# USCCACS/RXMD

Hardware: AMD Instinct MI355X
Metric: MD steps/sec (RDX, 979,776 atoms/GPU; one step advances every GPU's domain: weak scaling, wall-clock steps/s of the whole job) (higher is better)
Workload: dtype f64

## Files before the change

### rxmd_amd/csrc/nonbonded.hip

```cpp
#include "engine.h"

#include <cstdlib>

namespace rxmd {

static inline int nblk(long long n, int b) { return n > 0 ? static_cast<int>((n + b - 1) / b) : 1; }
static constexpr double CEchrge = 23.02;

__global__ void k_sorted_charge(int G, const int *__restrict__ rootperm, const double *__restrict__ q, double4 *__restrict__ pk) {
  const int k = blockIdx.x * blockDim.x + threadIdx.x;
  if (k < G) pk[k].w = q[rootperm[k]];
}

__device__ inline double wave_sum_n(double v) { return wave_sum64(v); }

struct NbAcc { double f0, f1, f2, v0, v1, v2, v3, v4, v5, e11, e12; };
template <bool ENERGY>
__device__ inline void nb_pair(const DevFF &ff, const int *__restrict__ ix2, double xi, double yi, double zi, double qi, const double4 &pj, int tj, NbAcc &a) {
  const double d0 = xi - pj.x, d1 = yi - pj.y, d2 = zi - pj.z;
  const double r2 = d0 * d0 + d1 * d1 + d2 * d2;
  if (r2 > ff.rctap2) return;
  const int inxn = ix2[tj];
  const int itb = static_cast<int>(r2 * ff.UDRi);
  double t = r2 - itb * ff.UDR;
  t = t * ff.UDRi;
  const DevNBTab nd = ff.tabNB[static_cast<size_t>(inxn) * (NTABLE + 2) + itb];
  const double qij = qi * pj.w;
  const double CEvdw = nd.CEvdw + t * nd.dCEvdw_;
  const double CEclmb = (nd.CEclmb + t * nd.dCEclmb_) * qij;
  if (ENERGY) {
    a.e11 += 0.5 * (nd.Evdw + t * nd.dEvdw_);
    a.e12 += 0.5 * (nd.Eclmb + t * nd.dEclmb_) * qij;
  }
  const double c = CEvdw + CEclmb;
  a.f0 -= c * d0; a.f1 -= c * d1; a.f2 -= c * d2;
  const double hc = -0.5 * c;
  a.v0 += hc * d0 * d0; a.v1 += hc * d1 * d1; a.v2 += hc * d2 * d2; a.v3 += hc * d1 * d2; a.v4 += hc * d2 * d0; a.v5 += hc * d0 * d1;
}

#ifndef NB_UNR
#define NB_UNR 8
#endif
#ifndef NB_WPB
#define NB_WPB 8
#endif
template <bool ENERGY>
__global__ void __launch_bounds__(64 * NB_WPB) k_nonbond(int N, int S10, DevFF ff, const int *__restrict__ nb10, const int *__restrict__ n10,
                                                  const double4 *__restrict__ pk, const double *__restrict__ x, const double *__restrict__ y, const double *__restrict__ z,
                                                  const double *__restrict__ q, const int *__restrict__ type,
                                                  double *__restrict__ fx, double *__restrict__ fy, double *__restrict__ fz, double *__restrict__ pe, int assign) {
  __shared__ double sm[NB_WPB][3], sv[NB_WPB][6];
  const int lane = threadIdx.x & 63, w = __builtin_amdgcn_readfirstlane(static_cast<int>(threadIdx.x >> 6));
  if (threadIdx.x < 6 * NB_WPB) sv[threadIdx.x / 6][threadIdx.x % 6] = 0.0;
  __syncthreads();
  const int i = xcd_swizzle(blockIdx.x, gridDim.x) * (blockDim.x >> 6) + w;
  double e11 = 0.0, e12 = 0.0, e13 = 0.0;
  if (i < N) {
    const double xi = x[i], yi = y[i], zi = z[i], qi = q[i];
    const int ti = type[i];
    const int n = n10[i] & N10_COUNT;
    const size_t row = static_cast<size_t>(i) * S10;
    const int *ix2 = ff.inxn2 + ti * ff.n1;
    NbAcc acc = {0.0, 0.0, 0.0, 0.0, 0.0, 0.0, 0.0, 0.0, 0.0, 0.0, 0.0};
    for (int k0 = lane; k0 < n; k0 += 64 * NB_UNR) {
      unsigned ee[NB_UNR];
#pragma unroll
      for (int u = 0; u < NB_UNR; ++u) { const int k = k0 + 64 * u; ee[u] = (k < n) ? static_cast<unsigned>(__builtin_nontemporal_load(nb10 + row + k)) : NB10_SELF; }
#pragma unroll
      for (int u = 0; u < NB_UNR; ++u) {
        const unsigned e = ee[u];
        if (e & NB10_SELF) continue;
        nb_pair<ENERGY>(ff, ix2, xi, yi, zi, qi, pk[e & NB10_IDX_MASK], static_cast<int>((e >> NB10_IDX_BITS) & 15u), acc);
      }
    }
    e11 = acc.e11; e12 = acc.e12;
    double f0 = wave_sum_n(acc.f0), f1 = wave_sum_n(acc.f1), f2 = wave_sum_n(acc.f2);
    double v0 = acc.v0, v1 = acc.v1, v2 = acc.v2, v3 = acc.v3, v4 = acc.v4, v5 = acc.v5;
    v0 = wave_sum_n(v0); v1 = wave_sum_n(v1); v2 = wave_sum_n(v2); v3 = wave_sum_n(v3); v4 = wave_sum_n(v4); v5 = wave_sum_n(v5);
    if (lane == 0) {
      if (assign) { fx[i] = f0; fy[i] = f1; fz[i] = f2; }
      else { fx[i] += f0; fy[i] += f1; fz[i] += f2; }
      if (ENERGY) { const DevAtomP ap = ff.atom[ti]; e13 = CEchrge * (ap.chi * qi + 0.5 * ap.eta * qi * qi); }
      sv[w][0] = v0 - xi * f0; sv[w][1] = v1 - yi * f1; sv[w][2] = v2 - zi * f2; sv[w][3] = v3 - yi * f2; sv[w][4] = v4 - zi * f0; sv[w][5] = v5 - xi * f1;
    }
  }
  if (ENERGY) {
    e11 = wave_sum_n(e11); e12 = wave_sum_n(e12); e13 = wave_sum_n(e13);
    if (lane == 0) { sm[w][0] = e11; sm[w][1] = e12; sm[w][2] = e13; }
  }
  __syncthreads();
  if (ENERGY && threadIdx.x < 3) {
    double s = 0.0;
    for (int k = 0; k < NB_WPB; ++k) s += sm[k][threadIdx.x];
    if (s != 0.0) atomicAdd(pe + 11 + threadIdx.x, s);
  }
  if (threadIdx.x >= 64 && threadIdx.x < 70) {
    const int c = threadIdx.x - 64;
    double s = 0.0;
    for (int k = 0; k < NB_WPB; ++k) s += sv[k][c];
    if (s != 0.0) atomicAdd(pe + 16 + c, s);
  }
}

template <bool ENERGY>
__global__ void __launch_bounds__(64 * WIN_ROWS, 8) k_nonbond_win(int N, int G, int S10, DevFF ff, const unsigned short *__restrict__ sl10, const int *__restrict__ n10,
                                                                const int *__restrict__ rows_sorted, const int *__restrict__ win_k, const int *__restrict__ win_cnt, int maxunits,
                                                                const double4 *__restrict__ pk, const unsigned char *__restrict__ stype,
                                                                const double *__restrict__ x, const double *__restrict__ y, const double *__restrict__ z,
                                                                const double *__restrict__ q, const int *__restrict__ type,
                                                                double *__restrict__ fx, double *__restrict__ fy, double *__restrict__ fz, double *__restrict__ pe, int assign) {
  extern __shared__ double4 s_p[];
  unsigned char *s_t = reinterpret_cast<unsigned char *>(s_p + static_cast<size_t>(maxunits) * WIN_UNIT);
  __shared__ double sm[WIN_ROWS][3], sv[WIN_ROWS][6];
  constexpr int NT = 64 * WIN_ROWS;
  const int lane = threadIdx.x & 63, w = __builtin_amdgcn_readfirstlane(static_cast<int>(threadIdx.x >> 6));
  const int grp = xcd_swizzle(blockIdx.x, gridDim.x);
  const int ridx = grp * WIN_ROWS + w;
  const int i = min(rows_sorted[ridx], N);
  const int nslots = WIN_UNIT * win_cnt[grp];
  const int *wk = win_k + static_cast<size_t>(grp) * WIN_MAXUNITS;
  const int capslots = WIN_UNIT * maxunits;
  for (int t = threadIdx.x; t < min(nslots, capslots); t += NT) {
    const int pos = min(wk[t / WIN_UNIT] + (t & (WIN_UNIT - 1)), G - 1);
    s_p[t] = pk[pos]; s_t[t] = stype[pos];
  }
  if (threadIdx.x < 6 * WIN_ROWS) sv[threadIdx.x / 6][threadIdx.x % 6] = 0.0;
  __syncthreads();
  double e11 = 0.0, e12 = 0.0, e13 = 0.0;
  if (i < N) {
    const double xi = x[i], yi = y[i], zi = z[i], qi = q[i];
    const int ti = type[i];
    const int n = n10[i] & N10_COUNT;
    const size_t row = static_cast<size_t>(i) * S10;
    const int *ix2 = ff.inxn2 + ti * ff.n1;
    NbAcc acc = {0.0, 0.0, 0.0, 0.0, 0.0, 0.0, 0.0, 0.0, 0.0, 0.0, 0.0};
    for (int k0 = lane; k0 < n; k0 += 64 * NB_UNR) {
      unsigned ee[NB_UNR];
#pragma unroll
      for (int u = 0; u < NB_UNR; ++u) { const int k = k0 + 64 * u; ee[u] = (k < n) ? static_cast<unsigned>(__builtin_nontemporal_load(sl10 + row + k)) : 0xffffu; }
#pragma unroll
      for (int u = 0; u < NB_UNR; ++u) {
        if (ee[u] == 0xffffu) continue;
        const int sl = static_cast<int>(ee[u] & 0x7fffu);
        if (sl < capslots) nb_pair<ENERGY>(ff, ix2, xi, yi, zi, qi, s_p[sl], static_cast<int>(s_t[sl]), acc);
        else { const int pos = min(wk[sl / WIN_UNIT] + (sl & (WIN_UNIT - 1)), G - 1); nb_pair<ENERGY>(ff, ix2, xi, yi, zi, qi, pk[pos], static_cast<int>(stype[pos]), acc); }
      }
    }
    e11 = acc.e11; e12 = acc.e12;
    const double f0 = wave_sum_n(acc.f0), f1 = wave_sum_n(acc.f1), f2 = wave_sum_n(acc.f2);
    const double v0 = wave_sum_n(acc.v0), v1 = wave_sum_n(acc.v1), v2 = wave_sum_n(acc.v2), v3 = wave_sum_n(acc.v3), v4 = wave_sum_n(acc.v4), v5 = wave_sum_n(acc.v5);
    if (lane == 0) {
      if (assign) { fx[i] = f0; fy[i] = f1; fz[i] = f2; }
      else { fx[i] += f0; fy[i] += f1; fz[i] += f2; }
      if (ENERGY) { const DevAtomP ap = ff.atom[ti]; e13 = CEchrge * (ap.chi * qi + 0.5 * ap.eta * qi * qi); }
      sv[w][0] = v0 - xi * f0; sv[w][1] = v1 - yi * f1; sv[w][2] = v2 - zi * f2; sv[w][3] = v3 - yi * f2; sv[w][4] = v4 - zi * f0; sv[w][5] = v5 - xi * f1;
    }
  }
  if (ENERGY) {
    e11 = wave_sum_n(e11); e12 = wave_sum_n(e12); e13 = wave_sum_n(e13);
    if (lane == 0) { sm[w][0] = e11; sm[w][1] = e12; sm[w][2] = e13; }
  }
  __syncthreads();
  if (ENERGY && threadIdx.x < 3) {
    double s = 0.0;
    for (int k = 0; k < WIN_ROWS; ++k) s += sm[k][threadIdx.x];
    if (s != 0.0) atomicAdd(pe + 11 + threadIdx.x, s);
  }
  if (threadIdx.x >= 64 && threadIdx.x < 70) {
    const int c = threadIdx.x - 64;
    double s = 0.0;
    for (int k = 0; k < WIN_ROWS; ++k) s += sv[k][c];
    if (s != 0.0) atomicAdd(pe + 16 + c, s);
  }
}

void Engine::sorted_charge_only() { k_sorted_charge<<<nblk(G, 256), 256, 0, stream>>>(G, multi() ? perm : rootperm, q, sorted_xyzi); sorted_w_charge = true; }
void Engine::charge_halo() {
  sorted_w_charge = true;
  if (multi()) {
    halo_staged(q, 1);
    k_sorted_charge<<<nblk(G, 256), 256, 0, stream>>>(G, perm, q, sorted_xyzi);
  } else
    k_sorted_charge<<<nblk(G, 256), 256, 0, stream>>>(G, rootperm, q, sorted_xyzi);
}

void Engine::nonbonded(bool to_fnb, bool energy) {
  double *f0 = to_fnb ? fnb[0] : frc[0], *f1 = to_fnb ? fnb[1] : frc[1], *f2 = to_fnb ? fnb[2] : frc[2];
  const int assign = to_fnb ? 1 : 0;
  const bool win_env = opt.nonbond_win != 0;
  const int units = std::min(win_maxunits, 296);
  const size_t lds = static_cast<size_t>(units) * WIN_UNIT * (sizeof(double4) + 1) + 16;
  if (win_valid && win_env && !list_selfcheck) {
#define RX_NB_WIN(EN) k_nonbond_win<EN><<<win_groups, 64 * WIN_ROWS, lds, stream>>>(N, G, S10, dff, sl10, n10, rows_sorted, win_k, win_cnt, units, sorted_xyzi, sorted_type, pos[0], pos[1], pos[2], q, type, \
                                                                 f0, f1, f2, scal + 32, assign)
    if (energy) RX_NB_WIN(true); else RX_NB_WIN(false);
#undef RX_NB_WIN
    RX_HIP(hipGetLastError());
    return;
  }
  require_nb10();
  if (energy) k_nonbond<true><<<nblk(N, NB_WPB), 64 * NB_WPB, 0, stream>>>(N, S10, dff, nb10, n10, sorted_xyzi, pos[0], pos[1], pos[2], q, type, f0, f1, f2, scal + 32, assign);
  else k_nonbond<false><<<nblk(N, NB_WPB), 64 * NB_WPB, 0, stream>>>(N, S10, dff, nb10, n10, sorted_xyzi, pos[0], pos[1], pos[2], q, type, f0, f1, f2, scal + 32, assign);
}

}
```

Before: 23.69.

## Compute nonbonded virial only for ghost pairs and skip it for interior rows

Reformulates the per-pair virial so it only accumulates for pairs whose neighbor is a ghost atom, using a midpoint-position form in place of the old full-pair virial minus an r_i·F correction. Rows and window groups flagged as having no ghost neighbors run a template variant with no virial accumulation, no virial wave reductions and no virial atomics; in force-only passes such blocks return early. The aim is to cut FP64 arithmetic, register pressure and reductions in the hot nonbonded loop. It depends on ghost flags (NB10_GHOST, N10_GHOST_ROW, sl10 bit 15, win_flag) that must be produced elsewhere, and the changed virial formulation could shift floating-point results.

```diff
diff --git a/rxmd_amd/csrc/nonbonded.hip b/rxmd_amd/csrc/nonbonded.hip
--- a/rxmd_amd/csrc/nonbonded.hip
+++ b/rxmd_amd/csrc/nonbonded.hip
@@ -1,6 +1,7 @@
 #include "engine.h"
 
 #include <cstdlib>
+#include <type_traits>
 
 namespace rxmd {
 
@@ -15,8 +16,8 @@
 __device__ inline double wave_sum_n(double v) { return wave_sum64(v); }
 
 struct NbAcc { double f0, f1, f2, v0, v1, v2, v3, v4, v5, e11, e12; };
-template <bool ENERGY>
-__device__ inline void nb_pair(const DevFF &ff, const int *__restrict__ ix2, double xi, double yi, double zi, double qi, const double4 &pj, int tj, NbAcc &a) {
+template <bool ENERGY, bool VIR>
+__device__ inline void nb_pair(const DevFF &ff, const int *__restrict__ ix2, double xi, double yi, double zi, double qi, const double4 &pj, int tj, bool ghost, NbAcc &a) {
   const double d0 = xi - pj.x, d1 = yi - pj.y, d2 = zi - pj.z;
   const double r2 = d0 * d0 + d1 * d1 + d2 * d2;
   if (r2 > ff.rctap2) return;
@@ -33,9 +34,13 @@
     a.e12 += 0.5 * (nd.Eclmb + t * nd.dEclmb_) * qij;
   }
   const double c = CEvdw + CEclmb;
-  a.f0 -= c * d0; a.f1 -= c * d1; a.f2 -= c * d2;
-  const double hc = -0.5 * c;
-  a.v0 += hc * d0 * d0; a.v1 += hc * d1 * d1; a.v2 += hc * d2 * d2; a.v3 += hc * d1 * d2; a.v4 += hc * d2 * d0; a.v5 += hc * d0 * d1;
+  a.f0 = __builtin_fma(-c, d0, a.f0); a.f1 = __builtin_fma(-c, d1, a.f1); a.f2 = __builtin_fma(-c, d2, a.f2);
+  if (VIR) {
+    const double cg = ghost ? c : 0.0;
+    const double t0 = cg * d0, t1 = cg * d1, t2 = cg * d2;
+    const double m0 = xi - 0.5 * d0, m1 = yi - 0.5 * d1, m2 = zi - 0.5 * d2;
+    a.v0 += t0 * m0; a.v1 += t1 * m1; a.v2 += t2 * m2; a.v3 += t2 * m1; a.v4 += t0 * m2; a.v5 += t1 * m0;
+  }
 }
 
 #ifndef NB_UNR
@@ -58,31 +63,38 @@
   if (i < N) {
     const double xi = x[i], yi = y[i], zi = z[i], qi = q[i];
     const int ti = type[i];
-    const int n = n10[i] & N10_COUNT;
+    const int nw = n10[i];
+    const int n = nw & N10_COUNT;
     const size_t row = static_cast<size_t>(i) * S10;
     const int *ix2 = ff.inxn2 + ti * ff.n1;
-    NbAcc acc = {0.0, 0.0, 0.0, 0.0, 0.0, 0.0, 0.0, 0.0, 0.0, 0.0, 0.0};
-    for (int k0 = lane; k0 < n; k0 += 64 * NB_UNR) {
-      unsigned ee[NB_UNR];
-#pragma unroll
-      for (int u = 0; u < NB_UNR; ++u) { const int k = k0 + 64 * u; ee[u] = (k < n) ? static_cast<unsigned>(__builtin_nontemporal_load(nb10 + row + k)) : NB10_SELF; }
-#pragma unroll
-      for (int u = 0; u < NB_UNR; ++u) {
-        const unsigned e = ee[u];
-        if (e & NB10_SELF) continue;
-        nb_pair<ENERGY>(ff, ix2, xi, yi, zi, qi, pk[e & NB10_IDX_MASK], static_cast<int>((e >> NB10_IDX_BITS) & 15u), acc);
-      }
-    }
-    e11 = acc.e11; e12 = acc.e12;
-    double f0 = wave_sum_n(acc.f0), f1 = wave_sum_n(acc.f1), f2 = wave_sum_n(acc.f2);
-    double v0 = acc.v0, v1 = acc.v1, v2 = acc.v2, v3 = acc.v3, v4 = acc.v4, v5 = acc.v5;
-    v0 = wave_sum_n(v0); v1 = wave_sum_n(v1); v2 = wave_sum_n(v2); v3 = wave_sum_n(v3); v4 = wave_sum_n(v4); v5 = wave_sum_n(v5);
-    if (lane == 0) {
-      if (assign) { fx[i] = f0; fy[i] = f1; fz[i] = f2; }
-      else { fx[i] += f0; fy[i] += f1; fz[i] += f2; }
-      if (ENERGY) { const DevAtomP ap = ff.atom[ti]; e13 = CEchrge * (ap.chi * qi + 0.5 * ap.eta * qi * qi); }
-      sv[w][0] = v0 - xi * f0; sv[w][1] = v1 - yi * f1; sv[w][2] = v2 - zi * f2; sv[w][3] = v3 - yi * f2; sv[w][4] = v4 - zi * f0; sv[w][5] = v5 - xi * f1;
-    }
+    auto whole = [&](auto vir) {
+      constexpr bool VIR = decltype(vir)::value;
+      NbAcc acc = {0.0, 0.0, 0.0, 0.0, 0.0, 0.0, 0.0, 0.0, 0.0, 0.0, 0.0};
+      for (int k0 = lane; k0 < n; k0 += 64 * NB_UNR) {
+        unsigned ee[NB_UNR];
+#pragma unroll
+        for (int u = 0; u < NB_UNR; ++u) { const int k = k0 + 64 * u; ee[u] = (k < n) ? static_cast<unsigned>(__builtin_nontemporal_load(nb10 + row + k)) : NB10_SELF; }
+#pragma unroll
+        for (int u = 0; u < NB_UNR; ++u) {
+          const unsigned e = ee[u];
+          if (e & NB10_SELF) continue;
+          nb_pair<ENERGY, VIR>(ff, ix2, xi, yi, zi, qi, pk[e & NB10_IDX_MASK], static_cast<int>((e >> NB10_IDX_BITS) & 15u), (e & NB10_GHOST) != 0u, acc);
+        }
+      }
+      e11 = acc.e11; e12 = acc.e12;
+      const double f0 = wave_sum_n(acc.f0), f1 = wave_sum_n(acc.f1), f2 = wave_sum_n(acc.f2);
+      double v0 = 0.0, v1 = 0.0, v2 = 0.0, v3 = 0.0, v4 = 0.0, v5 = 0.0;
+      if (VIR) {
+        v0 = wave_sum_n(acc.v0); v1 = wave_sum_n(acc.v1); v2 = wave_sum_n(acc.v2); v3 = wave_sum_n(acc.v3); v4 = wave_sum_n(acc.v4); v5 = wave_sum_n(acc.v5);
+      }
+      if (lane == 0) {
+        if (assign) { fx[i] = f0; fy[i] = f1; fz[i] = f2; }
+        else { fx[i] += f0; fy[i] += f1; fz[i] += f2; }
+        if (ENERGY) { const DevAtomP ap = ff.atom[ti]; e13 = CEchrge * (ap.chi * qi + 0.5 * ap.eta * qi * qi); }
+        if (VIR) { sv[w][0] = v0; sv[w][1] = v1; sv[w][2] = v2; sv[w][3] = v3; sv[w][4] = v4; sv[w][5] = v5; }
+      }
+    };
+    if (nw & N10_GHOST_ROW) whole(std::true_type{}); else whole(std::false_type{});
   }
   if (ENERGY) {
     e11 = wave_sum_n(e11); e12 = wave_sum_n(e12); e13 = wave_sum_n(e13);
@@ -104,7 +116,7 @@
 
 template <bool ENERGY>
 __global__ void __launch_bounds__(64 * WIN_ROWS, 8) k_nonbond_win(int N, int G, int S10, DevFF ff, const unsigned short *__restrict__ sl10, const int *__restrict__ n10,
-                                                                const int *__restrict__ rows_sorted, const int *__restrict__ win_k, const int *__restrict__ win_cnt, int maxunits,
+                                                                const int *__restrict__ rows_sorted, const int *__restrict__ win_k, const int *__restrict__ win_cnt, const int *__restrict__ win_flag, int maxunits,
                                                                 const double4 *__restrict__ pk, const unsigned char *__restrict__ stype,
                                                                 const double *__restrict__ x, const double *__restrict__ y, const double *__restrict__ z,
                                                                 const double *__restrict__ q, const int *__restrict__ type,
@@ -118,14 +130,17 @@
   const int ridx = grp * WIN_ROWS + w;
   const int i = min(rows_sorted[ridx], N);
   const int nslots = WIN_UNIT * win_cnt[grp];
+  const bool vir = ENERGY || win_flag[grp] != 0;
   const int *wk = win_k + static_cast<size_t>(grp) * WIN_MAXUNITS;
   const int capslots = WIN_UNIT * maxunits;
   for (int t = threadIdx.x; t < min(nslots, capslots); t += NT) {
     const int pos = min(wk[t / WIN_UNIT] + (t & (WIN_UNIT - 1)), G - 1);
     s_p[t] = pk[pos]; s_t[t] = stype[pos];
   }
-  if (threadIdx.x < 6 * WIN_ROWS) sv[threadIdx.x / 6][threadIdx.x % 6] = 0.0;
-  __syncthreads();
+  if (vir && threadIdx.x < 6 * WIN_ROWS) sv[threadIdx.x / 6][threadIdx.x % 6] = 0.0;
+  __syncthreads();
+  auto whole = [&](auto virc) {
+  constexpr bool VIR = decltype(virc)::value;
   double e11 = 0.0, e12 = 0.0, e13 = 0.0;
   if (i < N) {
     const double xi = x[i], yi = y[i], zi = z[i], qi = q[i];
@@ -142,20 +157,25 @@
       for (int u = 0; u < NB_UNR; ++u) {
         if (ee[u] == 0xffffu) continue;
         const int sl = static_cast<int>(ee[u] & 0x7fffu);
-        if (sl < capslots) nb_pair<ENERGY>(ff, ix2, xi, yi, zi, qi, s_p[sl], static_cast<int>(s_t[sl]), acc);
-        else { const int pos = min(wk[sl / WIN_UNIT] + (sl & (WIN_UNIT - 1)), G - 1); nb_pair<ENERGY>(ff, ix2, xi, yi, zi, qi, pk[pos], static_cast<int>(stype[pos]), acc); }
+        const bool gh = (ee[u] & 0x8000u) != 0u;
+        if (sl < capslots) nb_pair<ENERGY, VIR>(ff, ix2, xi, yi, zi, qi, s_p[sl], static_cast<int>(s_t[sl]), gh, acc);
+        else { const int pos = min(wk[sl / WIN_UNIT] + (sl & (WIN_UNIT - 1)), G - 1); nb_pair<ENERGY, VIR>(ff, ix2, xi, yi, zi, qi, pk[pos], static_cast<int>(stype[pos]), gh, acc); }
       }
     }
     e11 = acc.e11; e12 = acc.e12;
     const double f0 = wave_sum_n(acc.f0), f1 = wave_sum_n(acc.f1), f2 = wave_sum_n(acc.f2);
-    const double v0 = wave_sum_n(acc.v0), v1 = wave_sum_n(acc.v1), v2 = wave_sum_n(acc.v2), v3 = wave_sum_n(acc.v3), v4 = wave_sum_n(acc.v4), v5 = wave_sum_n(acc.v5);
+    double v0 = 0.0, v1 = 0.0, v2 = 0.0, v3 = 0.0, v4 = 0.0, v5 = 0.0;
+    if (VIR) {
+      v0 = wave_sum_n(acc.v0); v1 = wave_sum_n(acc.v1); v2 = wave_sum_n(acc.v2); v3 = wave_sum_n(acc.v3); v4 = wave_sum_n(acc.v4); v5 = wave_sum_n(acc.v5);
+    }
     if (lane == 0) {
       if (assign) { fx[i] = f0; fy[i] = f1; fz[i] = f2; }
       else { fx[i] += f0; fy[i] += f1; fz[i] += f2; }
       if (ENERGY) { const DevAtomP ap = ff.atom[ti]; e13 = CEchrge * (ap.chi * qi + 0.5 * ap.eta * qi * qi); }
-      sv[w][0] = v0 - xi * f0; sv[w][1] = v1 - yi * f1; sv[w][2] = v2 - zi * f2; sv[w][3] = v3 - yi * f2; sv[w][4] = v4 - zi * f0; sv[w][5] = v5 - xi * f1;
+      if (VIR) { sv[w][0] = v0; sv[w][1] = v1; sv[w][2] = v2; sv[w][3] = v3; sv[w][4] = v4; sv[w][5] = v5; }
     }
   }
+  if (!ENERGY && !VIR) return;
   if (ENERGY) {
     e11 = wave_sum_n(e11); e12 = wave_sum_n(e12); e13 = wave_sum_n(e13);
     if (lane == 0) { sm[w][0] = e11; sm[w][1] = e12; sm[w][2] = e13; }
@@ -166,12 +186,14 @@
     for (int k = 0; k < WIN_ROWS; ++k) s += sm[k][threadIdx.x];
     if (s != 0.0) atomicAdd(pe + 11 + threadIdx.x, s);
   }
-  if (threadIdx.x >= 64 && threadIdx.x < 70) {
+  if (VIR && threadIdx.x >= 64 && threadIdx.x < 70) {
     const int c = threadIdx.x - 64;
     double s = 0.0;
     for (int k = 0; k < WIN_ROWS; ++k) s += sv[k][c];
     if (s != 0.0) atomicAdd(pe + 16 + c, s);
   }
+  };
+  if (vir) whole(std::true_type{}); else whole(std::false_type{});
 }
 
 void Engine::sorted_charge_only() { k_sorted_charge<<<nblk(G, 256), 256, 0, stream>>>(G, multi() ? perm : rootperm, q, sorted_xyzi); sorted_w_charge = true; }
@@ -191,7 +213,7 @@
   const int units = std::min(win_maxunits, 296);
   const size_t lds = static_cast<size_t>(units) * WIN_UNIT * (sizeof(double4) + 1) + 16;
   if (win_valid && win_env && !list_selfcheck) {
-#define RX_NB_WIN(EN) k_nonbond_win<EN><<<win_groups, 64 * WIN_ROWS, lds, stream>>>(N, G, S10, dff, sl10, n10, rows_sorted, win_k, win_cnt, units, sorted_xyzi, sorted_type, pos[0], pos[1], pos[2], q, type, \
+#define RX_NB_WIN(EN) k_nonbond_win<EN><<<win_groups, 64 * WIN_ROWS, lds, stream>>>(N, G, S10, dff, sl10, n10, rows_sorted, win_k, win_cnt, win_flag, units, sorted_xyzi, sorted_type, pos[0], pos[1], pos[2], q, type, \
                                                                  f0, f1, f2, scal + 32, assign)
     if (energy) RX_NB_WIN(true); else RX_NB_WIN(false);
 #undef RX_NB_WIN
```

Result: no change. 23.63 (-0.3%).
